# lmchion/PowerGridworld

Hardware: AMD Instinct MI355X
Metric: agent-env-steps/sec at batch 65536, 5-agent scenario, 1/2/4/8 MI355X (higher is better)
Workload: dtype f64; 1 GPU; C4: 5-agent coordinated buildings (building+PV+storage) + IEEE-13 power flow + voltage-violation reward; pf_convergence=opendss, batch_per_gpu=65536, global_batch=65536, episode_steps=286, parallelism=env-sharded x1 (no collective on the step path)

## Files before the change

include/pgw.h:

```cpp
#ifndef PGW_H_
#define PGW_H_

#include <stdint.h>

#ifdef __cplusplus
extern "C" {
#endif

#define PGW_ABI_VERSION 31

#define PGW_OK 0
#define PGW_ERR_ARG (-1)
#define PGW_ERR_HIP (-2)

int32_t pgw_abi_version(void);
const char* pgw_last_error(void);

#define PGW_N_STRUCT_SIZES 30
int32_t pgw_struct_sizes(int64_t* out, int32_t n);

typedef struct pgw_mat {
  double* ptr;
  int64_t s_env;
  int64_t s_dim;
} pgw_mat;

typedef struct pgw_matf {
  float* ptr;
  int64_t s_env;
  int64_t s_dim;
} pgw_matf;

#define PGW_OOB_EPS 1e-4

typedef struct pgw_battery_params {
  double soc_min, soc_max;
  double eta_c, eta_d;
  double max_power;
  double dt_h;
  int32_t rescale;
  int32_t sampled_init;
// ... 196 lines not shown
  const double* start;
  const double* resp;
  double resp_x0, resp_h;
  int32_t resp_nseg;
  int32_t resp_v_row;
  const double* resp_v;
  uint64_t resp_rows;
  const double* resp_q;
  uint64_t resp_q_rows;
  int32_t resp_q_stride, resp_q_k;
} pgw_pf_od;

int32_t pgw_pf_solve(const pgw_pf_params* p, const pgw_pf_tables* t, int64_t n,
                     const double* ctrl_p, const double* ctrl_q, double* v_out,
                     int32_t* iters, void* stream);
int32_t pgw_pf_solve_f32(const pgw_pf_params* p, const pgw_pf_tables* t, int64_t n,
                         const float* ctrl_p, const float* ctrl_q, float* v_out,
                         int32_t* iters, void* stream);

int64_t pgw_pf_od_probe_args_size(int32_t n_hours);
int32_t pgw_pf_od_probe(const pgw_pf_params* p_hours, int32_t n_hours, const pgw_pf_tables* t,
                        const double* start_h, int32_t lanes_per_hour, int64_t n, const double* P,
                        double* J_out, uint64_t* sig_out, int32_t* it_out, void* args_buf, void* stream);

int32_t pgw_pf_od_resp_fit(int32_t m, int64_t n_pieces, const double* J, const int32_t* idx3,
                           const double* meta, const int32_t* inext, const int32_t* rec, double* out,
                           void* stream);

int32_t pgw_pf_od_resp_check(int32_t m, int64_t n, const double* recs, const int32_t* rec, const double* P,
                             const double* J, const int32_t* iq, double* err, void* stream);

int32_t pgw_pf_pred_pack(const pgw_pf_params* p, int32_t n_tables, int32_t n_points,
                         const double* U_grid, double* rec, void* stream);
int32_t pgw_pf_pred_meta(const pgw_pf_params* p, int32_t n_tables, int32_t n_points,
                         const double* U_pred, const int32_t* sig, pgw_pred_meta* meta,
                         void* stream);

int32_t pgw_voltage_band_penalty(int64_t n, const double* v, double lo, double hi, double scale,
                                 double* out, void* stream);

int32_t pgw_pf_padded_m(int32_t m);
int64_t pgw_pf_pack_size(int32_t m);
int32_t pgw_pf_pack(const pgw_pf_params* p, const double* W, const double* U0, const double* G0,
                    const double* V0_0, double* out);

#define PGW_PFG_MAX_M 128
// ... 384 lines not shown
```

powergridworld_amd/_lib.py:

```python
import ctypes as C
import os

import torch

_HERE = os.path.dirname(os.path.abspath(__file__))
LIB_PATH = os.environ.get("PGW_LIB_PATH") or os.path.join(_HERE, "libpgw.so")
ABI_VERSION = 31

f64, i32, i64, u64, vp = C.c_double, C.c_int32, C.c_int64, C.c_uint64, C.c_void_p
P = C.POINTER

BLD_MAX_OBS = 24
EV_MAX_WORDS = 16
MAX_COMP = 8
PF_MAX_M = 16
PF_MAX_CTRL = 8
PFG_MAX_M = 128
PFG_MAX_CHK = 256
MAX_AGENTS = 8


class PgwError(RuntimeError):
    pass


class Mat(C.Structure):
    _fields_ = [("ptr", vp), ("s_env", i64), ("s_dim", i64)]


class Matf(C.Structure):
# ... 229 lines not shown
                ("soc_min", f64), ("soc_max", f64), ("eta_c", f64), ("eta_d", f64), ("max_power", f64),
                ("dt_h", f64), ("max_storage_cost", f64),
                ("ev_rate", f64), ("ev_hours_per_step", f64), ("ev_steps_per_hour", f64), ("ev_mult", f64),
                ("ev_unserved_penalty", f64), ("ev_obs_low", f64 * 7), ("ev_obs_high", f64 * 7),
                ("ev_end_park", f64 * HS_MAX_VEHICLES), ("ev_req0", f64 * HS_MAX_VEHICLES),
                ("dev_act_low", f64), ("dev_act_high", f64), ("dev_hours_per_step", f64),
                ("dev_obs_high", f64 * HS_MAX_DEV), ("max_grid_power", f64), ("oob", vp),
                ("pv_grid_aware", i32), ("pad_", i32)]


class HSStepInfo(C.Structure):
    _fields_ = [("pv_avail", f64), ("grid_cost", f64), ("dev_obs", f64 * HS_MAX_DEV),
                ("dev_power", f64 * HS_MAX_DEV), ("ev_time", f64), ("ev_next_time", f64),
                ("ev_window", C.c_uint64)]


class HSBuffers(C.Structure):
    _fields_ = [("action", Mat), ("obs", Mat), ("soc", vp), ("soc_cost", vp), ("ev_req", vp),
                ("ev_charging", vp), ("ev_cost", vp), ("dev_cost", vp), ("es_power_last", vp),
                ("reward", vp), ("real_power", vp), ("meta_out", vp), ("step_meta", vp),
                ("pv_power_last", vp), ("min_voltage", vp)]


PGW_ELEM_LINE, PGW_ELEM_XFMR, PGW_ELEM_VSOURCE, PGW_ELEM_SHUNT, PGW_ELEM_XFMR_N = 1, 2, 3, 4, 5

_SIGS = {
    "pgw_abi_version": (i32, []),
    "pgw_struct_sizes": (i32, [P(i64), i32]),
    "pgw_pf_od_probe_args_size": (i64, [i32]),
    "pgw_pf_od_probe": (i32, [P(PFParams), i32, P(PFTables), vp, i32, i64, vp, vp, vp, vp, vp, vp]),
    "pgw_pf_od_resp_fit": (i32, [i32, i64, vp, vp, vp, vp, vp, vp, vp]),
    "pgw_pf_od_resp_check": (i32, [i32, i64, vp, vp, vp, vp, vp, vp, vp]),
    "pgw_last_error": (C.c_char_p, []),
    "pgw_battery_reset": (i32, [P(BatteryParams), i64, vp, vp, Mat, vp]),
    "pgw_battery_step": (i32, [P(BatteryParams), i64, Mat, vp, Mat, vp, vp]),
    "pgw_battery_reset_f32": (i32, [P(BatteryParams), i64, vp, vp, Matf, vp]),
    "pgw_battery_step_f32": (i32, [P(BatteryParams), i64, Matf, vp, Matf, vp, vp]),
    "pgw_pv_obs": (i32, [P(PVParams), i64, f64, vp, Mat, vp]),
    "pgw_pv_step": (i32, [P(PVParams), i64, f64, Mat, vp, Mat, vp, vp]),
    "pgw_building_reset": (i32, [P(BuildingParams), P(BuildingExo), i64, vp, vp, vp, BuildingExt,
                                 Mat, vp]),
    "pgw_building_step": (i32, [P(BuildingParams), P(BuildingExo), P(BuildingExo), i64, Mat, vp, vp,
                                vp, vp, i32, BuildingExt, Mat, vp]),
    "pgw_ev_reset": (i32, [P(EVParams), i64, vp, vp, vp, vp]),
    "pgw_ev_reset_tables": (i32, [P(EVParams), i64, vp, vp, vp, vp]),
    "pgw_pv_obs_f32": (i32, [P(PVParams), i64, f64, vp, Matf, vp]),
    "pgw_pv_step_f32": (i32, [P(PVParams), i64, f64, Matf, vp, Matf, vp, vp]),
    "pgw_building_reset_f32": (i32, [P(BuildingParams), P(BuildingExo), i64, vp, vp, vp, BuildingExt, Matf, vp]),
    "pgw_building_step_f32": (i32, [P(BuildingParams), P(BuildingExo), P(BuildingExo), i64, Matf, vp, vp, vp, vp,
                                    i32, BuildingExt, Matf, vp]),
    "pgw_ev_reset_f32": (i32, [P(EVParams), i64, vp, vp, vp, vp]),
    "pgw_ev_reset_tables_f32": (i32, [P(EVParams), i64, vp, vp, vp, vp]),
    "pgw_ev_step_f32": (i32, [P(EVParams), P(EVStepInfo), i64, Matf, vp, vp, vp, Matf, vp, vp, vp]),
# ... 22 lines not shown
    "pgw_coord_step": (i32, [P(CoordParams), P(PFParams), P(PFTables), P(CoordStepInfo), i64,
                             CoordBuffers, vp]),
    "pgw_coord_step_f32": (i32, [P(CoordParams), P(PFParams), P(PFTables), P(CoordStepInfo), i64,
                                 CoordBuffersF32, vp]),
    "pgw_coord_step_general": (i32, [P(CoordParams), P(PFGParams), P(PFGTables), P(CoordStepInfo), i64,
                                     CoordBuffers, vp]),
    "pgw_hs_reset": (i32, [P(HSParams), P(HSStepInfo), i64, vp, HSBuffers, vp]),
    "pgw_mc_agent_step": (i32, [P(MCStepArgs), i64, vp]),
    "pgw_mc_agent_step_f32": (i32, [P(MCStepArgsF32), i64, vp]),
    "pgw_mc_ev_split_mode": (i32, [i32, P(i32)]),
    "pgw_graph_begin": (i32, [vp]),
    "pgw_graph_end": (i32, [vp, P(vp)]),
    "pgw_graph_launch": (i32, [vp, vp]),
    "pgw_graph_destroy": (i32, [vp]),
    "pgw_hs_step": (i32, [P(HSParams), P(HSStepInfo), i64, HSBuffers, vp]),
    "pgw_ma_step": (i32, [P(MAStepArgs), P(PFParams), P(PFTables), i64, vp, vp, vp]),
}

EXPORTED = sorted(_SIGS)

STRUCTS = [Mat, BatteryParams, PVParams, BuildingParams, BuildingExo, BuildingExt, EVParams,
           EVStepInfo, ReduceArgs, PFParams, PFTables, FeederElem, CoordParams, CoordBuffers,
           CoordStepInfo, PredMeta, HSParams, HSStepInfo, HSBuffers, MCStepArgs, Matf, CoordBuffersF32,
           MAStepArgs, PFGElem, PFGParams, PFGTables, RegParams, MCStepDyn, PFOD, MCStepArgsF32]

_lib = None


def lib():
    global _lib
    if _lib is not None:
        return _lib
    if not os.path.exists(LIB_PATH):
        raise PgwError("libpgw.so not found at %s -- build it with "
                       "`python -c 'import __graft_entry__ as g; g.build()'` or "
                       "`make -C powergridworld_amd/csrc`" % LIB_PATH)
    h = C.CDLL(LIB_PATH)
    for name, (res, args) in _SIGS.items():
        fn = getattr(h, name)
        fn.restype = res
        fn.argtypes = args
    if h.pgw_abi_version() != ABI_VERSION:
        raise PgwError("libpgw ABI %d != expected %d (rebuild)" % (h.pgw_abi_version(), ABI_VERSION))
    sizes = (i64 * len(STRUCTS))()
    h.pgw_struct_sizes(sizes, len(STRUCTS))
    for st, sz in zip(STRUCTS, sizes):
        if C.sizeof(st) != sz:
# ... 59 lines not shown
```

powergridworld_amd/csrc/pgw_feeder.cpp:

```cpp
#include <cmath>
#include <complex>
#include <cstdarg>
#include <cstdio>
#include <cstring>
#include <vector>

#include "pgw.h"

namespace pgw {
void set_error(const char* fmt, ...);
}

namespace {

using cplx = std::complex<double>;
using Mat = std::vector<cplx>;
using xcplx = std::complex<long double>;
using XMat = std::vector<xcplx>;

template <typename CT>
bool invert(std::vector<CT>& a, int n) {
  using R = typename CT::value_type;
  std::vector<CT> inv(static_cast<size_t>(n) * n, CT(0, 0));
  for (int i = 0; i < n; ++i) inv[i * n + i] = R(1);
// ... 208 lines not shown
  }
}

}

extern "C" {

int32_t pgw_struct_sizes(int64_t* out, int32_t n) {
  const int64_t sz[PGW_N_STRUCT_SIZES] = {
      (int64_t)sizeof(pgw_mat),           (int64_t)sizeof(pgw_battery_params),
      (int64_t)sizeof(pgw_pv_params),     (int64_t)sizeof(pgw_building_params),
      (int64_t)sizeof(pgw_building_exo),  (int64_t)sizeof(pgw_building_ext),
      (int64_t)sizeof(pgw_ev_params),     (int64_t)sizeof(pgw_ev_step_info),
      (int64_t)sizeof(pgw_reduce_args),   (int64_t)sizeof(pgw_pf_params),
      (int64_t)sizeof(pgw_pf_tables),     (int64_t)sizeof(pgw_feeder_elem),
      (int64_t)sizeof(pgw_coord_params),  (int64_t)sizeof(pgw_coord_buffers),
      (int64_t)sizeof(pgw_coord_step_info), (int64_t)sizeof(pgw_pred_meta),
      (int64_t)sizeof(pgw_hs_params),       (int64_t)sizeof(pgw_hs_step_info),
      (int64_t)sizeof(pgw_hs_buffers),      (int64_t)sizeof(pgw_mc_step_args),
      (int64_t)sizeof(pgw_matf),            (int64_t)sizeof(pgw_coord_buffers_f32),
      (int64_t)sizeof(pgw_ma_step_args),   (int64_t)sizeof(pgw_pfg_elem),
      (int64_t)sizeof(pgw_pfg_params),     (int64_t)sizeof(pgw_pfg_tables),
      (int64_t)sizeof(pgw_reg_params),    (int64_t)sizeof(pgw_mc_step_dyn),
      (int64_t)sizeof(pgw_pf_od),         (int64_t)sizeof(pgw_mc_step_args_f32)};
  for (int i = 0; i < n && i < PGW_N_STRUCT_SIZES; ++i) out[i] = sz[i];
  return PGW_N_STRUCT_SIZES;
}

int32_t pgw_feeder_build(const pgw_feeder_elem* elems, int32_t n_elems, int32_t n_nodes, double* Y,
                         double* Z, double* I_src, double* V0) {
  if (!elems || n_elems <= 0 || n_nodes <= 0) {
    pgw::set_error("pgw_feeder_build: empty feeder");
    return PGW_ERR_ARG;
  }
  try {
    Builder B(n_nodes);
    for (int i = 0; i < n_elems; ++i) {
      const pgw_feeder_elem& e = elems[i];
      if (e.nphases < 1 || e.nphases > 3) {
        pgw::set_error("pgw_feeder_build: element %d has %d phases", i, e.nphases);
        return PGW_ERR_ARG;
      }
      bool ok = false;
      switch (e.kind) {
        case PGW_ELEM_VSOURCE: ok = add_vsource(B, e); break;
        case PGW_ELEM_XFMR: ok = add_transformer(B, e); break;
        case PGW_ELEM_XFMR_N: ok = add_transformer_n(B, e); break;
// ... 99 lines not shown
```

powergridworld_amd/csrc/pgw_pf.hip:

```cpp
#include <algorithm>
#include <cstdlib>
#include <cmath>
#include <type_traits>
#include <atomic>
#include <vector>

#include "pgw_common.h"

static std::atomic<bool> g_pf_trace_on{false};

namespace pgw {

template <int B, int E, class F>
__device__ __forceinline__ void static_for(F&& f) {
  if constexpr (B < E) {
    f(std::integral_constant<int, B>{});
    static_for<B + 1, E>(f);
  }
}

template <int M> struct PFBlock {
  static constexpr int kTri = M * (M + 1) / 2;
  static constexpr int kU0re = 3 * kTri, kU0im = kU0re + M, kU0sum = kU0im + M;
  static constexpr int kLo2 = kU0sum + M, kMn2 = kLo2 + M, kMx2 = kMn2 + M;
  static constexpr int kG0re = kMx2 + M, kG0im = kG0re + M, kV0re = kG0im + M, kV0im = kV0re + 1;
  static constexpr int kSize = kV0im + 1;
  static constexpr int kPairs = (kSize + 15) / 16;
};
static int64_t pf_block_size(int m) { return 3LL * m * (m + 1) / 2 + 8LL * m + 2; }

// ... 2175 lines not shown
  __shared__ ODShared<M> sh;
  ODStage<M> stg;
  od_stage_load<M>(o, start, stg);
  PFSolver<M, true, false> S;
  S.load(a, t.block);
  double cp[PGW_PF_MAX_CTRL], cq[PGW_PF_MAX_CTRL];
#pragma unroll
  for (int c = 0; c < PGW_PF_MAX_CTRL; ++c) {
    cp[c] = (valid && c == 0) ? P[e] : 0.0;
    cq[c] = 0.0;
  }
  S.powers(a, cp, cq, 1.0);
  od_stage_store<M>(o, stg, sh);
  __syncthreads();
  uint64_t sig = kFnvBasis;
  const int it = od_solve<M, true>(S, o, stg, valid, sh, &sig);
  double ir[M], ii[M];
  od_load_J<M>(sh, it, ir, ii);
  if (!valid) return;
#pragma unroll
  for (int k = 0; k < M; ++k) J_out[e * M + k] = make_double2(ir[k], ii[k]);
  sig_out[e] = sig;
  it_out[e] = it;
}

__global__ void __launch_bounds__(kBlock) k_pf_od_resp_fit(int32_t m, int64_t np, const double2* __restrict__ J,
                                                           const int32_t* __restrict__ idx3,
                                                           const double* __restrict__ meta,
                                                           const int32_t* __restrict__ inext,
                                                           const int32_t* __restrict__ rec, double* __restrict__ out) {
  const int64_t i = (int64_t)blockIdx.x * kBlock + threadIdx.x;
  if (i >= np) return;
  double* o = out + (int64_t)rec[i] * PGW_OD_REC(m);
  for (int q = 0; q < 4; ++q) o[q] = meta[4 * i + q];
  const unsigned long long packed =
      (unsigned long long)(uint32_t)inext[2 * i] | ((unsigned long long)(uint32_t)inext[2 * i + 1] << 32);
  o[4] = __longlong_as_double((long long)packed);
  o[5] = 0.0;
  const double2* ja = J + (int64_t)idx3[3 * i] * m;
  const double2* jm = J + (int64_t)idx3[3 * i + 1] * m;
  const double2* jb = J + (int64_t)idx3[3 * i + 2] * m;
  double* c = o + PGW_OD_REC_HEAD;
  for (int k = 0; k < m; ++k) {
    const double2 a = ja[k], md = jm[k], b = jb[k];
    c[2 * k] = md.x;
    c[2 * k + 1] = md.y;
// ... 465 lines not shown
  PGW_REQUIRE(n_hours >= 1 && n >= 0 && lanes_per_hour > 0 && lanes_per_hour % kBlock == 0 &&
              n <= (int64_t)n_hours * lanes_per_hour,
              "pgw_pf_od_probe: n %lld lanes over %d hours of %d (a multiple of %d)", (long long)n, n_hours,
              lanes_per_hour, kBlock);
  std::vector<PFArgs> args(n_hours);
  for (int h = 0; h < n_hours; ++h) {
    const int32_t rc = check_od(p_hours[h], *t, "pgw_pf_od_probe");
    if (rc) return rc;
    PGW_REQUIRE(p_hours[h].m == p_hours[0].m && p_hours[h].n_ctrl == p_hours[0].n_ctrl &&
                p_hours[h].max_iter == p_hours[0].max_iter, "pgw_pf_od_probe: hours differ in shape");
    args[h] = make_pf_args(p_hours[h], *t);
  }
  if (n == 0) return PGW_OK;
  hipStream_t st = (hipStream_t)stream;
  PGW_REQUIRE(hipMemcpyAsync(args_buf, args.data(), sizeof(PFArgs) * n_hours, hipMemcpyHostToDevice, st) ==
                  hipSuccess && hipStreamSynchronize(st) == hipSuccess,
              "pgw_pf_od_probe: argument upload failed");
  hipLaunchKernelGGL(k_pf_od_probe<14>, dim3(grid_for(n)), dim3(kBlock), 0, st,
                     reinterpret_cast<const PFArgs*>(args_buf), make_od_args(*t->od, p_hours[0].max_iter), *t,
                     start_h, lanes_per_hour, n, P, reinterpret_cast<double2*>(J_out), sig_out, it_out);
  return check_launch("k_pf_od_probe");
}

int32_t pgw_pf_od_resp_fit(int32_t m, int64_t n_pieces, const double* J, const int32_t* idx3,
                           const double* meta, const int32_t* inext, const int32_t* rec, double* out,
                           void* stream) {
  PGW_REQUIRE(m >= 1 && m <= PGW_PF_MAX_M && n_pieces >= 0, "pgw_pf_od_resp_fit: bad m / n_pieces");
  if (n_pieces == 0) return PGW_OK;
  PGW_REQUIRE(J && idx3 && meta && inext && rec && out, "pgw_pf_od_resp_fit: null argument");
  hipLaunchKernelGGL(k_pf_od_resp_fit, dim3(grid_for(n_pieces)), dim3(kBlock), 0, (hipStream_t)stream, m,
                     n_pieces, reinterpret_cast<const double2*>(J), idx3, meta, inext, rec, out);
  return check_launch("k_pf_od_resp_fit");
}

int32_t pgw_pf_od_resp_check(int32_t m, int64_t n, const double* recs, const int32_t* rec, const double* P,
                             const double* J, const int32_t* iq, double* err, void* stream) {
  PGW_REQUIRE(m >= 1 && m <= PGW_PF_MAX_M && n >= 0, "pgw_pf_od_resp_check: bad m / n");
  if (n == 0) return PGW_OK;
  PGW_REQUIRE(recs && rec && P && J && iq && err, "pgw_pf_od_resp_check: null argument");
  hipLaunchKernelGGL(k_pf_od_resp_check, dim3(grid_for(n)), dim3(kBlock), 0, (hipStream_t)stream, m, n, recs,
                     rec, P, reinterpret_cast<const double2*>(J), iq, err);
  return check_launch("k_pf_od_resp_check");
}

int32_t pgw_pf_pred_meta(const pgw_pf_params* p, int32_t n_tables, int32_t n_points,
                         const double* U_pred, const int32_t* sig, pgw_pred_meta* meta,
// ... 137 lines not shown
```

powergridworld_amd/distribution_system/od_certify.py:

```python
import numpy as np
import torch

FNV_BASIS = np.uint64(0xcbf29ce484222325)
FNV_PRIME = np.uint64(0x100000001b3)


class SnapModel:

    def __init__(self, u1b, u1P, J0, jP, s0, fr, y0, u0, W, G, V0, lo2, mn2, mx2, tol, min_iter, max_iter):
        self.u1b, self.u1P, self.J0, self.jP = u1b, u1P, J0, jP
        self.s0, self.fr, self.y0, self.u0 = s0, fr, y0, u0
        self.W, self.G, self.V0 = W, G, V0
        self.Wa, self.Ga = W.abs(), G.abs()
        self.lo2, self.mn2, self.mx2 = float(lo2), float(mn2), float(mx2)
        self.tol, self.min_iter, self.max_iter = float(tol), int(min_iter), int(max_iter)

    @property
    def M(self):
        return self.u0.shape[0]

    @classmethod
    def from_solver(cls, s, rows, hours):
        M, dev = s.M, s.device
        st = s._od_start[torch.as_tensor(rows, device=dev)].to(torch.float64)
        c = torch.view_as_complex(st.reshape(len(rows), 6, M, 2).contiguous())
        p0, od = s.params, s._od_proto
        nph = np.array(p0.nph[:M])
        ctrl0 = np.array(p0.elem_ctrl[:M]) == 0
        s0 = []
        for h in hours:
            p = s._params_for_hour(h)
            s0.append((np.array(p.base_kw[:M]) * 1000.0) / nph - 1j * ((np.array(p.base_kvar[:M]) * 1000.0) / nph))
        T = lambda a: torch.as_tensor(np.ascontiguousarray(a), device=dev)
        return cls(u1b=c[:, 0], u1P=c[0, 1], J0=c[:, 3], jP=c[0, 4], s0=T(np.array(s0)),
                   fr=T(np.where(ctrl0, 1000.0 / nph, 0.0)),
                   y0=T(np.array(od.y0r[:M]) + 1j * np.array(od.y0i[:M])), u0=T(s._od_u0),
                   W=T(s._od_W2), G=T(s._od_Gall[:, :M]), V0=T(s._od_V0all),
                   lo2=p0.vlow[0] ** 2, mn2=p0.vmin[0] ** 2, mx2=p0.vmax[0] ** 2,
# ... 78 lines not shown
    rem = torch.where(gap > 0, e + ba * ba / (2.0 * torch.where(gap > 0, gap, torch.ones_like(gap))),
                      torch.full_like(aa, float("inf")))
    return aa, slope, rem


def _mul_cr(sa, sb, g0, g1, eg):
    a = sa * g0
    b = sa * g1 + sb * g0
    e = sb.abs() * g1.abs() + (sa.abs() + sb.abs()) * eg
    return a, b, e


def _mul_cc(x, y):
    xa, xb, xe = x
    ya, yb, ye = y
    a = xa * ya
    b = xa * yb + xb * ya
    e = xb.abs() * yb.abs() + (xa.abs() + xb.abs()) * ye + (ya.abs() + yb.abs()) * xe + xe * ye
    return a, b, e


def certify(model, h, lo, hi, delta_band=1e-12, delta_stop=1e-12):
    dev = model.u0.device
    h = torch.as_tensor(h, device=dev)
    lo = torch.as_tensor(lo, dtype=torch.float64, device=dev)
    hi = torch.as_tensor(hi, dtype=torch.float64, device=dev)
    K, M = lo.shape[0], model.M
    c, r = (0.5 * (lo + hi))[:, None], (0.5 * (hi - lo))[:, None]
    zero_e = torch.zeros((K, M), dtype=torch.float64, device=dev)
    u = (model.u1b[h] + c * model.u1P, r * model.u1P, zero_e)
    Jp = (model.J0[h] + c * model.jP, r * model.jP, zero_e)
    Vp = _lin(Jp, model.G, model.Ga, model.V0)
    s_a = model.s0[h] + (c * model.fr).to(torch.complex128)
    s_b = (r * model.fr).to(torch.complex128)
    ok = torch.ones(K, dtype=torch.bool, device=dev)
    done = torch.zeros(K, dtype=torch.bool, device=dev)
    conv = torch.zeros_like(done)
    its = torch.ones(K, dtype=torch.int64, device=dev)
    shifts = 2 * torch.arange(M, device=dev)
    thr = (model.lo2, model.mn2, model.mx2)
    bands = []
    for it in range(2, model.max_iter + 1):
        m0, m1, em, mlo, mhi = _mag2(u)
        b = torch.zeros((K, M), dtype=torch.int64, device=dev)
        for T in thr:
            above, below = mlo > T + delta_band, mhi < T - delta_band
            ok &= done | (above | below).all(1)
            b += above.long()
        bands.append(torch.where(done, -1, (b << shifts).sum(1)))
        inband = b == 2
        safe = torch.where(inband, m0, torch.ones_like(m0))
        g0 = torch.where(inband, 1.0 / safe,
                         torch.where(b == 1, 1.0 / model.mn2, torch.where(b == 3, 1.0 / model.mx2, 1.0)))
        g1 = torch.where(inband, -m1 / (safe * safe), torch.zeros_like(m1))
        mlo_s = torch.where(inband, mlo, torch.ones_like(mlo))
        eg = torch.where(inband, em / (safe * safe) + (m1.abs() + em) ** 2 / (safe * safe * mlo_s),
                         torch.zeros_like(em))
        ok &= done | torch.isfinite(eg).all(1)
        ya, yb, ye = _mul_cr(s_a, s_b, g0, g1, eg)
        J = _mul_cc((ya - model.y0, yb, ye), u)
        V = _lin(J, model.G, model.Ga, model.V0)
        un = _lin(J, model.W, model.Wa, model.u0)
        n0, n1, nr = _mag(V)
        p0, p1, pr = _mag(Vp)
        d0, d1, dr = n0 - p0, n1 - p1, nr + pr
        dlo, dhi = d0 - d1.abs() - dr, d0 + d1.abs() + dr
        amax = torch.maximum(dlo.abs(), dhi.abs())
        amin = torch.where((dlo <= 0) & (dhi >= 0), torch.zeros_like(dlo), torch.minimum(dlo.abs(), dhi.abs()))
        if it >= model.min_iter:
            yes = (amax <= model.tol - delta_stop).all(1)
            no = (amin > model.tol + delta_stop).any(1)
        else:
            yes = torch.zeros_like(done)
            no = torch.ones_like(done)
        ok &= done | yes | no
        its = torch.where(done, its, torch.full_like(its, it))
        conv |= ~done & yes
        done = done | yes | (it >= model.max_iter) | ~ok
        u = tuple(torch.where(done[:, None], x_o, x_n) for x_o, x_n in zip(u, un))
        Vp = V
        if bool(done.all()):
            break
    ret = torch.where(conv, its, -its)
    return ok.cpu().numpy(), ret.cpu().numpy(), signature(torch.stack(bands, 1), ret)


def certify_pieces(model, h, a, b, it, sig, min_width=1e-9, max_depth=12, max_live=64, split=16):
    h, a, b = np.asarray(h), np.asarray(a, float), np.asarray(b, float)
    it, sig = np.asarray(it, np.int64), np.asarray(sig, np.uint64)
    n = len(a)
    out_lo, out_hi, kw = np.full(n, np.inf), np.full(n, -np.inf), np.zeros(n)
    if n == 0:
        return out_lo, out_hi, kw
    owner, lo, hi = np.arange(n), a.copy(), b.copy()
    good = {}
    for level in range(max_depth):
        if not len(owner):
            break
        ok, ret, sg = certify(model, h[owner], lo, hi)
        ok &= (ret == it[owner]) & (sg == sig[owner])
        if level == 0:
            out_lo[ok], out_hi[ok], kw[ok] = a[ok], b[ok], b[ok] - a[ok]
        else:
            for q in np.nonzero(ok)[0]:
                good.setdefault(owner[q], []).append((lo[q], hi[q]))
        bad = np.nonzero(~ok & (hi - lo > split * min_width))[0]
        if max_live:
# ... 26 lines not shown
```

powergridworld_amd/distribution_system/opendss.py:

```python
import os
from datetime import datetime
from typing import List, Union

import numpy as np
import pandas as pd
import torch

from powergridworld_amd import _lib
from powergridworld_amd.base import as_env_tensor
from powergridworld_amd.distribution_system.feeder import DATA_DIR, Feeder, load_feeder_spec
from powergridworld_amd.distribution_system.powerflow import PowerFlowSolver

PHASE_MAP = {'a': '.1', 'b': '.2', 'c': '.3'}


def bus_name_to_nodes(bus_name: str) -> List[str]:
    if bus_name[-1] in PHASE_MAP.keys():
        return [bus_name.replace(bus_name[-1], PHASE_MAP[bus_name[-1]])]
    return [bus_name + p for p in PHASE_MAP.values()]


def load_loadshape(loadshape_file):
    base = os.path.basename(str(loadshape_file)).lower()
    if base == "annual_hourly_load_profile.csv" and not os.path.exists(str(loadshape_file)):
# ... 221 lines not shown
        od.gamma = max([float(np.abs(Gs[j] - Gs[r]).max()) for j, r in members], default=0.0)
        od.eps = max([float(abs(V0s[j] - V0s[r])) for j, r in members], default=0.0)
        od.gmax = float(rowmax[elem_nodes + reps].max())
        od.gsrc = float(rowmax[src].max()) if src else 0.0
        dev = self.device
        cdev = lambda a: torch.tensor(np.ascontiguousarray(a).view(np.float64).ravel(), dtype=torch.float64,
                                      device=dev)
        self._od_Gall, self._od_V0all = Gs, V0s
        self._od_rows_V0 = cdev(V0s[rows] if rows else np.zeros(1, complex))
        self._od_rows_G = cdev(Gs[rows] if rows else np.zeros((1, M), complex))
        od.rows_V0, od.rows_G = self._od_rows_V0.data_ptr(), self._od_rows_G.data_ptr()
        self._od_proto = od
        self._od_rows = [f.node_names[i] for i in rows]
        self._od_W2 = W / (vb_elem[:, None] * vb_elem[None, :])
        self._od_u0 = U0 / vb_elem
        self._od_start = torch.zeros((self.OD_MAX_TABLES, 12 * M), dtype=torch.float64, device=dev)
        self._od_resp = None
        self._od_vresp = None
        self._od_rowmask = {}
        self.od_node_records = True
        self.od_row_masks = True
        self.od_record_rows = True
        self.od_certify = True
        self.od_row_records = True
        self._od_qrec = None
        self._od_qinfo = {}
        self._od_qflags = {}
        self.od_resp_stats, self.od_resp_brackets = {}, {}
        self._od_index = {}
        self._od_keep = {}

    def _od_starts(self, hour):
        hours, keys = [], []
        for h in range(hour, min(hour + self.PREDICTOR_LOOKAHEAD, len(self.annual_hourly_load_profile))):
            k = self._hour_key(h)
            if k not in self._od_index and k not in keys:
                hours.append(h)
                keys.append(k)
        if len(self._od_index) + len(keys) > self.OD_MAX_TABLES:
            self._od_index, self._tables_cache, self._od_keep = {}, {}, {}
            self.tables_version += 1
        idx0 = len(self._od_index)
        M, od = self.M, self._od_proto
        W2, u0 = self._od_W2, self._od_u0
        p0 = self.params
        nph = np.array(p0.nph[:M])
# ... 310 lines not shown
        err = torch.empty(2 * len(pa), dtype=torch.float64, device=dev)
        dr, dp, dq_ = T(np.repeat(prec, 2), np.int32), T(chk.ravel(), np.float64), T(c_l.ravel(), np.int32)
        _lib.check(lib.pgw_pf_od_resp_check(M, 2 * len(pa), self._od_resp.data_ptr(), dr.data_ptr(), dp.data_ptr(),
                                            Jc.data_ptr(), dq_.data_ptr(), err.data_ptr(), st))
        e_ = err.cpu().numpy().reshape(-1, 2).max(1)
        del dr, dp, dq_
        vnode = self._od_vnode()
        if vnode is not None and len(pa):
            rr = self._od_resp.view(-1, R)[torch.from_numpy(prec).to(dev)]
            vc = self._od_vcoef(rr)
            tt = (torch.from_numpy(chk).to(dev) - rr[:, 2:3]) * rr[:, 3:4]
            vfit = vc[:, :1] + tt * (vc[:, 1:2] + tt * vc[:, 2:3])
            Jl = torch.view_as_complex(Jc.reshape(-1, M, 2)[torch.from_numpy(c_l.ravel()).to(dev)].contiguous())
            G = torch.from_numpy(np.ascontiguousarray(self._od_Gall[vnode, :M])).to(dev)
            vtrue = ((Jl * G).sum(-1) + complex(self._od_V0all[vnode])).reshape(-1, 2)
            ev = ((vfit - vtrue).abs() / vtrue.abs()).max(1).values.cpu().numpy()
            e_ = np.maximum(e_, np.where(np.isfinite(ev), ev, np.inf))
        bad = (pit != 0) & ((e_ > self.OD_RESP_TOL) | (sc[c_l] != psig[:, None]).any(1) | ~np.isfinite(e_))
        cand = np.nonzero((pit != 0) & ~bad)[0]
        n_cut, kw_cut, t_cert = 0, 0.0, _time.perf_counter()
        if self.od_certify and len(cand):
            from powergridworld_amd.distribution_system.od_certify import SnapModel, certify_pieces
            model = SnapModel.from_solver(self, list(range(idx0, idx0 + H)), hours)
            c_lo, c_hi, c_kw = certify_pieces(model, pq_[cand], pa[cand], pb[cand], pit[cand], psig[cand],
                                              min_width=self.OD_RESP_MIN_WIDTH)
            none = c_lo > c_hi
            bad[cand[none]] = True
            cut = ~none & ((c_lo > pa[cand]) | (c_hi < pb[cand]))
            n_cut = int(cut.sum())
            kw_cut = float(((pb - pa)[cand] - np.where(none, 0.0, c_hi - c_lo)).sum())
            if n_cut:
                hdr = torch.from_numpy(np.stack([c_lo[cut], c_hi[cut]], 1)).to(dev)
                self._od_resp.view(-1, R)[torch.from_numpy(prec[cand[cut]]).to(dev), 0:2] = hdr
        t_cert = _time.perf_counter() - t_cert
        if bad.any():
            words = np.array([self._od_meta_word(0, int(nx)) for nx in pnext[bad]], np.int64)
            self._od_resp.view(-1, R).view(torch.int64)[torch.from_numpy(prec[bad]).to(dev), 4] = \
                torch.from_numpy(words).to(dev)
        ok = (pit != 0) & ~bad
        if vnode is not None:
            if self._od_vresp is None:
                self._od_vresp = torch.zeros((self.OD_MAX_TABLES, rec_n, _lib.OD_VREC), dtype=torch.float64,
                                             device=dev)
            vb = self._od_vresp[idx0:idx0 + H]
            vb.view(torch.int64)[:, :, :6] = blk.view(torch.int64)[:, :, :6]
            vb[:, :, 6:12] = torch.view_as_real(self._od_vcoef(blk)).reshape(H, rec_n, 6)
# ... 639 lines not shown
```

Before: 15.65 billion agent-env-steps/s.

## Port interval power-flow certification to a fused native HIP kernel

Adds a HIP kernel that runs the per-interval affine-arithmetic fixed-point certification entirely per lane, with per-node previous magnitudes kept in LDS. It replaces the iterative PyTorch implementation, which launched many small tensor ops per iteration, whenever the model lives on a GPU. The certification runs during OpenDSS response-table construction, not inside the per-step environment kernel. So any gain shows up only through table-building overhead that is amortized over steps. It adds an ABI bump and a hardcoded m=14, and results could differ slightly from the torch path.

```diff
diff --git a/include/pgw.h b/include/pgw.h
--- a/include/pgw.h
+++ b/include/pgw.h
@@ -7,7 +7,7 @@
 extern "C" {
 #endif
 
-#define PGW_ABI_VERSION 31
+#define PGW_ABI_VERSION 32
 
 #define PGW_OK 0
 #define PGW_ERR_ARG (-1)
@@ -16,7 +16,7 @@
 int32_t pgw_abi_version(void);
 const char* pgw_last_error(void);
 
-#define PGW_N_STRUCT_SIZES 30
+#define PGW_N_STRUCT_SIZES 31
 int32_t pgw_struct_sizes(int64_t* out, int32_t n);
 
 typedef struct pgw_mat {
@@ -259,6 +259,16 @@
 int32_t pgw_pf_od_probe(const pgw_pf_params* p_hours, int32_t n_hours, const pgw_pf_tables* t,
                         const double* start_h, int32_t lanes_per_hour, int64_t n, const double* P,
                         double* J_out, uint64_t* sig_out, int32_t* it_out, void* args_buf, void* stream);
+
+typedef struct pgw_od_certify_model {
+  const double *u1b, *u1P, *J0, *jP, *s0, *fr, *y0, *u0, *W, *Wa, *G, *Ga, *V0;
+  double lo2, mn2, mx2, tol, delta_band, delta_stop;
+  int32_t m, n_nodes, n_hours, min_iter, max_iter, pad_;
+} pgw_od_certify_model;
+#define PGW_OD_CERTIFY_MAX_NODES 42
+
+int32_t pgw_pf_od_certify(const pgw_od_certify_model* model, int64_t k, const int32_t* h, const double* lo,
+                          const double* hi, int32_t* ok, int32_t* ret, uint64_t* sig, void* stream);
 
 int32_t pgw_pf_od_resp_fit(int32_t m, int64_t n_pieces, const double* J, const int32_t* idx3,
                            const double* meta, const int32_t* inext, const int32_t* rec, double* out,
diff --git a/powergridworld_amd/_lib.py b/powergridworld_amd/_lib.py
--- a/powergridworld_amd/_lib.py
+++ b/powergridworld_amd/_lib.py
@@ -5,7 +5,7 @@
 
 _HERE = os.path.dirname(os.path.abspath(__file__))
 LIB_PATH = os.environ.get("PGW_LIB_PATH") or os.path.join(_HERE, "libpgw.so")
-ABI_VERSION = 31
+ABI_VERSION = 32
 
 f64, i32, i64, u64, vp = C.c_double, C.c_int32, C.c_int64, C.c_uint64, C.c_void_p
 P = C.POINTER
@@ -281,6 +281,14 @@
                 ("pv_power_last", vp), ("min_voltage", vp)]
 
 
+class ODCertifyModel(C.Structure):
+    _fields_ = [(k, vp) for k in ("u1b", "u1P", "J0", "jP", "s0", "fr", "y0", "u0", "W", "Wa", "G", "Ga", "V0")] + \
+               [(k, f64) for k in ("lo2", "mn2", "mx2", "tol", "delta_band", "delta_stop")] + \
+               [(k, i32) for k in ("m", "n_nodes", "n_hours", "min_iter", "max_iter", "pad_")]
+
+
+OD_CERTIFY_MAX_NODES = 42
+
 PGW_ELEM_LINE, PGW_ELEM_XFMR, PGW_ELEM_VSOURCE, PGW_ELEM_SHUNT, PGW_ELEM_XFMR_N = 1, 2, 3, 4, 5
 
 _SIGS = {
@@ -288,6 +296,7 @@
     "pgw_struct_sizes": (i32, [P(i64), i32]),
     "pgw_pf_od_probe_args_size": (i64, [i32]),
     "pgw_pf_od_probe": (i32, [P(PFParams), i32, P(PFTables), vp, i32, i64, vp, vp, vp, vp, vp, vp]),
+    "pgw_pf_od_certify": (i32, [P(ODCertifyModel), i64, vp, vp, vp, vp, vp, vp, vp]),
     "pgw_pf_od_resp_fit": (i32, [i32, i64, vp, vp, vp, vp, vp, vp, vp]),
     "pgw_pf_od_resp_check": (i32, [i32, i64, vp, vp, vp, vp, vp, vp, vp]),
     "pgw_last_error": (C.c_char_p, []),
@@ -356,7 +365,8 @@
 STRUCTS = [Mat, BatteryParams, PVParams, BuildingParams, BuildingExo, BuildingExt, EVParams,
            EVStepInfo, ReduceArgs, PFParams, PFTables, FeederElem, CoordParams, CoordBuffers,
            CoordStepInfo, PredMeta, HSParams, HSStepInfo, HSBuffers, MCStepArgs, Matf, CoordBuffersF32,
-           MAStepArgs, PFGElem, PFGParams, PFGTables, RegParams, MCStepDyn, PFOD, MCStepArgsF32]
+           MAStepArgs, PFGElem, PFGParams, PFGTables, RegParams, MCStepDyn, PFOD, MCStepArgsF32,
+           ODCertifyModel]
 
 _lib = None
 
diff --git a/powergridworld_amd/csrc/pgw_feeder.cpp b/powergridworld_amd/csrc/pgw_feeder.cpp
--- a/powergridworld_amd/csrc/pgw_feeder.cpp
+++ b/powergridworld_amd/csrc/pgw_feeder.cpp
@@ -254,7 +254,8 @@
       (int64_t)sizeof(pgw_ma_step_args),   (int64_t)sizeof(pgw_pfg_elem),
       (int64_t)sizeof(pgw_pfg_params),     (int64_t)sizeof(pgw_pfg_tables),
       (int64_t)sizeof(pgw_reg_params),    (int64_t)sizeof(pgw_mc_step_dyn),
-      (int64_t)sizeof(pgw_pf_od),         (int64_t)sizeof(pgw_mc_step_args_f32)};
+      (int64_t)sizeof(pgw_pf_od),         (int64_t)sizeof(pgw_mc_step_args_f32),
+      (int64_t)sizeof(pgw_od_certify_model)};
   for (int i = 0; i < n && i < PGW_N_STRUCT_SIZES; ++i) out[i] = sz[i];
   return PGW_N_STRUCT_SIZES;
 }
diff --git a/powergridworld_amd/csrc/pgw_od_certify.h b/powergridworld_amd/csrc/pgw_od_certify.h
--- /dev/null
+++ b/powergridworld_amd/csrc/pgw_od_certify.h
@@ -0,0 +1,176 @@
+#pragma once
+#include <math.h>
+#include <stdint.h>
+
+#include "pgw.h"
+
+#ifdef __HIPCC__
+#define PGW_CERT_HD __host__ __device__ __forceinline__
+#else
+#define PGW_CERT_HD inline
+#endif
+
+PGW_CERT_HD double cert_max(double x, double y) { return (x != x || y != y) ? NAN : (x > y ? x : y); }
+PGW_CERT_HD double cert_min(double x, double y) { return (x != x || y != y) ? NAN : (x < y ? x : y); }
+
+PGW_CERT_HD void cert_mag(double ar, double ai, double br, double bi, double e, double& m0, double& m1,
+                          double& rem) {
+#pragma clang fp contract(off)
+  const double aa = hypot(ar, ai), ba = hypot(br, bi);
+  m1 = (ar * br + ai * bi) / (aa > 0.0 ? aa : 1.0);
+  const double gap = aa - ba;
+  rem = gap > 0.0 ? e + ba * ba / (2.0 * gap) : (double)INFINITY;
+  m0 = aa;
+}
+
+template <int M>
+PGW_CERT_HD void cert_row(const double* __restrict__ mat, const double* __restrict__ mabs,
+                          const double* __restrict__ cst, int n, const double* xar, const double* xai,
+                          const double* xbr, const double* xbi, const double* xe, double& ar, double& ai,
+                          double& br, double& bi, double& e) {
+#pragma clang fp contract(off)
+  const double* g = mat + 2 * (int64_t)n * M;
+  const double* ga = mabs + (int64_t)n * M;
+  double sar = 0.0, sai = 0.0, sbr = 0.0, sbi = 0.0, se = 0.0;
+#pragma unroll
+  for (int j = 0; j < M; ++j) {
+    const double gr = g[2 * j], gi = g[2 * j + 1];
+    sar += xar[j] * gr - xai[j] * gi;
+    sai += xar[j] * gi + xai[j] * gr;
+    sbr += xbr[j] * gr - xbi[j] * gi;
+    sbi += xbr[j] * gi + xbi[j] * gr;
+    se += xe[j] * ga[j];
+  }
+  ar = cst[2 * n] + sar;
+  ai = cst[2 * n + 1] + sai;
+  br = sbr;
+  bi = sbi;
+  e = se;
+}
+
+template <int M>
+PGW_CERT_HD void od_certify_lane(const pgw_od_certify_model& a, int h, double lo, double hi,
+                                 double* __restrict__ prev, int stride, int32_t* ok_out, int32_t* ret_out,
+                                 uint64_t* sig_out) {
+#pragma clang fp contract(off)
+  const int N = a.n_nodes;
+  const double c = 0.5 * (lo + hi), r = 0.5 * (hi - lo);
+  const double thr[3] = {a.lo2, a.mn2, a.mx2};
+  const double tol_yes = a.tol - a.delta_stop, tol_no = a.tol + a.delta_stop;
+  const double* u1b = a.u1b + 2 * (int64_t)h * M;
+  const double* J0 = a.J0 + 2 * (int64_t)h * M;
+  const double* s0 = a.s0 + 2 * (int64_t)h * M;
+  double uar[M], uai[M], ubr[M], ubi[M], ue[M];
+  double jar[M], jai[M], jbr[M], jbi[M], je[M];
+#pragma unroll
+  for (int k = 0; k < M; ++k) {
+    uar[k] = u1b[2 * k] + c * a.u1P[2 * k];
+    uai[k] = u1b[2 * k + 1] + c * a.u1P[2 * k + 1];
+    ubr[k] = r * a.u1P[2 * k];
+    ubi[k] = r * a.u1P[2 * k + 1];
+    ue[k] = 0.0;
+    jar[k] = J0[2 * k] + c * a.jP[2 * k];
+    jai[k] = J0[2 * k + 1] + c * a.jP[2 * k + 1];
+    jbr[k] = r * a.jP[2 * k];
+    jbi[k] = r * a.jP[2 * k + 1];
+    je[k] = 0.0;
+  }
+#pragma unroll 1
+  for (int n = 0; n < N; ++n) {
+    double var, vai, vbr, vbi, ve, p0, p1, pr;
+    cert_row<M>(a.G, a.Ga, a.V0, n, jar, jai, jbr, jbi, je, var, vai, vbr, vbi, ve);
+    cert_mag(var, vai, vbr, vbi, ve, p0, p1, pr);
+    prev[(3 * n + 0) * (int64_t)stride] = p0;
+    prev[(3 * n + 1) * (int64_t)stride] = p1;
+    prev[(3 * n + 2) * (int64_t)stride] = pr;
+  }
+  bool ok = true, conv = false;
+  int its = 1;
+  uint64_t sig = 0xcbf29ce484222325ull;
+  const uint64_t prime = 0x100000001b3ull;
+  for (int it = 2; it <= a.max_iter; ++it) {
+    uint64_t bands = 0;
+    bool certain = true;
+#pragma unroll
+    for (int k = 0; k < M; ++k) {
+      const double ar = uar[k], ai = uai[k], br = ubr[k], bi = ubi[k], e = ue[k];
+      const double m0 = ar * ar + ai * ai;
+      const double m1 = 2.0 * (ar * br + ai * bi);
+      const double q2 = br * br + bi * bi;
+      const double qmax = m0 + fabs(m1) + q2;
+      const double q2s = q2 > 0.0 ? q2 : 1.0;
+      const double tv = q2 > 0.0 ? -m1 / (2.0 * q2s) : 0.0;
+      const bool inside = q2 > 0.0 && fabs(tv) <= 1.0;
+      double qmin = inside ? m0 - m1 * m1 / (4.0 * q2s) : m0 - fabs(m1) + q2;
+      qmin = qmin < 0.0 ? 0.0 : qmin;
+      double rlo = sqrt(qmin) - e;
+      rlo = rlo < 0.0 ? 0.0 : rlo;
+      const double mlo = rlo * rlo;
+      const double rhi = sqrt(qmax) + e;
+      const double mhi = rhi * rhi;
+      const double aa = hypot(ar, ai), ba = hypot(br, bi);
+      const double em = q2 + 2.0 * (aa + ba) * e + e * e;
+      int b = 0;
+#pragma unroll
+      for (int q = 0; q < 3; ++q) {
+        const bool above = mlo > thr[q] + a.delta_band, below = mhi < thr[q] - a.delta_band;
+        certain &= above | below;
+        b += above ? 1 : 0;
+      }
+      bands |= (uint64_t)b << (2 * k);
+      const bool inband = b == 2;
+      const double safe = inband ? m0 : 1.0;
+      const double g0 = inband ? 1.0 / safe : (b == 1 ? 1.0 / a.mn2 : (b == 3 ? 1.0 / a.mx2 : 1.0));
+      const double g1 = inband ? -m1 / (safe * safe) : 0.0;
+      const double mlo_s = inband ? mlo : 1.0;
+      const double w = fabs(m1) + em;
+      const double eg = inband ? em / (safe * safe) + w * w / (safe * safe * mlo_s) : 0.0;
+      certain &= (bool)isfinite(eg);
+      const double sar = s0[2 * k] + c * a.fr[k], sai = s0[2 * k + 1] + 0.0, sbr = r * a.fr[k];
+      const double sa_abs = hypot(sar, sai), sb_abs = fabs(sbr);
+      const double yar = sar * g0 - a.y0[2 * k], yai = sai * g0 - a.y0[2 * k + 1];
+      const double ybr = sar * g1 + sbr * g0, ybi = sai * g1 + 0.0;
+      const double ye = sb_abs * fabs(g1) + (sa_abs + sb_abs) * eg;
+      jar[k] = yar * ar - yai * ai;
+      jai[k] = yar * ai + yai * ar;
+      jbr[k] = (yar * br - yai * bi) + (ybr * ar - ybi * ai);
+      jbi[k] = (yar * bi + yai * br) + (ybr * ai + ybi * ar);
+      const double ya_abs = hypot(yar, yai), yb_abs = hypot(ybr, ybi);
+      je[k] = yb_abs * ba + (ya_abs + yb_abs) * e + (aa + ba) * ye + ye * e;
+    }
+    ok &= certain;
+    sig = (sig ^ bands) * prime;
+    bool yes = true, no = false;
+#pragma unroll 1
+    for (int n = 0; n < N; ++n) {
+      double var, vai, vbr, vbi, ve, n0, n1, nr;
+      cert_row<M>(a.G, a.Ga, a.V0, n, jar, jai, jbr, jbi, je, var, vai, vbr, vbi, ve);
+      cert_mag(var, vai, vbr, vbi, ve, n0, n1, nr);
+      double* p = prev + 3 * n * (int64_t)stride;
+      const double d0 = n0 - p[0], d1 = n1 - p[stride], dr = nr + p[2 * (int64_t)stride];
+      const double dlo = d0 - fabs(d1) - dr, dhi = d0 + fabs(d1) + dr;
+      const double amax = cert_max(fabs(dlo), fabs(dhi));
+      const double amin = (dlo <= 0.0 && dhi >= 0.0) ? 0.0 : cert_min(fabs(dlo), fabs(dhi));
+      yes &= amax <= tol_yes;
+      no |= amin > tol_no;
+      p[0] = n0;
+      p[stride] = n1;
+      p[2 * (int64_t)stride] = nr;
+    }
+    if (it < a.min_iter) {
+      yes = false;
+      no = true;
+    }
+    ok &= yes | no;
+    its = it;
+    conv |= yes;
+    if (yes || it >= a.max_iter || !ok) break;
+#pragma unroll
+    for (int k = 0; k < M; ++k)
+      cert_row<M>(a.W, a.Wa, a.u0, k, jar, jai, jbr, jbi, je, uar[k], uai[k], ubr[k], ubi[k], ue[k]);
+  }
+  const int32_t ret = conv ? its : -its;
+  *ok_out = ok ? 1 : 0;
+  *ret_out = ret;
+  *sig_out = (sig ^ (uint64_t)(uint32_t)ret) * prime;
+}
diff --git a/powergridworld_amd/csrc/pgw_pf.hip b/powergridworld_amd/csrc/pgw_pf.hip
--- a/powergridworld_amd/csrc/pgw_pf.hip
+++ b/powergridworld_amd/csrc/pgw_pf.hip
@@ -6,6 +6,7 @@
 #include <vector>
 
 #include "pgw_common.h"
+#include "pgw_od_certify.h"
 
 static std::atomic<bool> g_pf_trace_on{false};
 
@@ -2227,6 +2228,27 @@
   for (int k = 0; k < M; ++k) J_out[e * M + k] = make_double2(ir[k], ii[k]);
   sig_out[e] = sig;
   it_out[e] = it;
+}
+
+constexpr int kCertBlock = 64;
+template <int M>
+__global__ void __launch_bounds__(kCertBlock) k_pf_od_certify(pgw_od_certify_model a, int64_t K,
+                                                              const int32_t* __restrict__ h,
+                                                              const double* __restrict__ lo,
+                                                              const double* __restrict__ hi,
+                                                              int32_t* __restrict__ ok, int32_t* __restrict__ ret,
+                                                              uint64_t* __restrict__ sig) {
+  extern __shared__ double cert_prev[];
+  const int64_t e = (int64_t)blockIdx.x * kCertBlock + threadIdx.x;
+  if (e >= K) return;
+  const int row = h[e];
+  if (row < 0 || row >= a.n_hours) {
+    ok[e] = 0;
+    ret[e] = 0;
+    sig[e] = 0;
+    return;
+  }
+  od_certify_lane<M>(a, row, lo[e], hi[e], cert_prev + threadIdx.x, kCertBlock, ok + e, ret + e, sig + e);
 }
 
 __global__ void __launch_bounds__(kBlock) k_pf_od_resp_fit(int32_t m, int64_t np, const double2* __restrict__ J,
@@ -2738,6 +2760,26 @@
   return check_launch("k_pf_od_probe");
 }
 
+int32_t pgw_pf_od_certify(const pgw_od_certify_model* model, int64_t k, const int32_t* h, const double* lo,
+                          const double* hi, int32_t* ok, int32_t* ret, uint64_t* sig, void* stream) {
+  PGW_REQUIRE(model && k >= 0, "pgw_pf_od_certify: null model / negative k");
+  const pgw_od_certify_model& a = *model;
+  PGW_REQUIRE(a.m == 14 && a.n_nodes >= 1 && a.n_nodes <= PGW_OD_CERTIFY_MAX_NODES && a.n_hours >= 1 &&
+              a.max_iter >= 2,
+              "pgw_pf_od_certify: m %d (14), n_nodes %d (1..%d), n_hours %d, max_iter %d (>= 2)", a.m, a.n_nodes,
+              PGW_OD_CERTIFY_MAX_NODES, a.n_hours, a.max_iter);
+  PGW_REQUIRE(a.u1b && a.u1P && a.J0 && a.jP && a.s0 && a.fr && a.y0 && a.u0 && a.W && a.Wa && a.G && a.Ga && a.V0,
+              "pgw_pf_od_certify: null model array");
+  if (k == 0) return PGW_OK;
+  PGW_REQUIRE(h && lo && hi && ok && ret && sig, "pgw_pf_od_certify: null argument");
+  const int64_t blocks = (k + kCertBlock - 1) / kCertBlock;
+  PGW_REQUIRE(blocks <= 0x7fffffffll, "pgw_pf_od_certify: %lld intervals", (long long)k);
+  const size_t lds = sizeof(double) * 3 * (size_t)a.n_nodes * kCertBlock;
+  hipLaunchKernelGGL(k_pf_od_certify<14>, dim3((unsigned)blocks), dim3(kCertBlock), lds, (hipStream_t)stream, a, k,
+                     h, lo, hi, ok, ret, sig);
+  return check_launch("k_pf_od_certify");
+}
+
 int32_t pgw_pf_od_resp_fit(int32_t m, int64_t n_pieces, const double* J, const int32_t* idx3,
                            const double* meta, const int32_t* inext, const int32_t* rec, double* out,
                            void* stream) {
diff --git a/powergridworld_amd/distribution_system/od_certify.py b/powergridworld_amd/distribution_system/od_certify.py
--- a/powergridworld_amd/distribution_system/od_certify.py
+++ b/powergridworld_amd/distribution_system/od_certify.py
@@ -14,6 +14,25 @@
         self.Wa, self.Ga = W.abs(), G.abs()
         self.lo2, self.mn2, self.mx2 = float(lo2), float(mn2), float(mx2)
         self.tol, self.min_iter, self.max_iter = float(tol), int(min_iter), int(max_iter)
+        self.native = True
+        self._native = None
+
+    def native_model(self, delta_band, delta_stop):
+        from powergridworld_amd import _lib
+        if self._native is None:
+            ri = lambda z: torch.view_as_real(z.to(torch.complex128).contiguous()).contiguous()
+            re = lambda x: x.to(torch.float64).contiguous()
+            arrays = dict(u1b=ri(self.u1b), u1P=ri(self.u1P), J0=ri(self.J0), jP=ri(self.jP), s0=ri(self.s0),
+                          fr=re(self.fr), y0=ri(self.y0), u0=ri(self.u0), W=ri(self.W), Wa=re(self.Wa),
+                          G=ri(self.G), Ga=re(self.Ga), V0=ri(self.V0))
+            m = _lib.ODCertifyModel(m=self.M, n_nodes=self.G.shape[0], n_hours=self.u1b.shape[0],
+                                    **{k: v.data_ptr() for k, v in arrays.items()})
+            self._native = (m, arrays)
+        m = self._native[0]
+        m.lo2, m.mn2, m.mx2, m.tol = self.lo2, self.mn2, self.mx2, self.tol
+        m.min_iter, m.max_iter = self.min_iter, self.max_iter
+        m.delta_band, m.delta_stop = float(delta_band), float(delta_stop)
+        return m
 
     @property
     def M(self):
@@ -138,6 +157,8 @@
 
 def certify(model, h, lo, hi, delta_band=1e-12, delta_stop=1e-12):
     dev = model.u0.device
+    if model.native and dev.type == "cuda":
+        return _certify_native(model, h, lo, hi, delta_band, delta_stop)
     h = torch.as_tensor(h, device=dev)
     lo = torch.as_tensor(lo, dtype=torch.float64, device=dev)
     hi = torch.as_tensor(hi, dtype=torch.float64, device=dev)
@@ -166,8 +187,9 @@
         bands.append(torch.where(done, -1, (b << shifts).sum(1)))
         inband = b == 2
         safe = torch.where(inband, m0, torch.ones_like(m0))
+        one = torch.ones_like(m0)
         g0 = torch.where(inband, 1.0 / safe,
-                         torch.where(b == 1, 1.0 / model.mn2, torch.where(b == 3, 1.0 / model.mx2, 1.0)))
+                         torch.where(b == 1, one * (1.0 / model.mn2), torch.where(b == 3, one * (1.0 / model.mx2), one)))
         g1 = torch.where(inband, -m1 / (safe * safe), torch.zeros_like(m1))
         mlo_s = torch.where(inband, mlo, torch.ones_like(mlo))
         eg = torch.where(inband, em / (safe * safe) + (m1.abs() + em) ** 2 / (safe * safe * mlo_s),
@@ -199,6 +221,27 @@
             break
     ret = torch.where(conv, its, -its)
     return ok.cpu().numpy(), ret.cpu().numpy(), signature(torch.stack(bands, 1), ret)
+
+
+def _certify_native(model, h, lo, hi, delta_band, delta_stop):
+    from powergridworld_amd import _lib
+    host = lambda x, dt: (x.detach().cpu().numpy() if torch.is_tensor(x) else np.asarray(x)).astype(dt)
+    h, lo, hi = host(h, np.int32), host(lo, np.float64), host(hi, np.float64)
+    K, dev = lo.shape[0], model.u0.device
+    if K == 0:
+        return np.zeros(0, bool), np.zeros(0, np.int64), np.zeros(0, np.uint64)
+    inp = np.empty((3, K), np.float64)
+    inp[0], inp[1] = lo, hi
+    inp[2].view(np.int32)[:K] = h
+    d_in = torch.from_numpy(inp).to(dev)
+    d_out = torch.empty((2, K), dtype=torch.int64, device=dev)
+    i32 = d_out[1].view(torch.int32)
+    _lib.check(_lib.lib().pgw_pf_od_certify(model.native_model(delta_band, delta_stop), K, d_in[2].data_ptr(),
+                                            d_in[0].data_ptr(), d_in[1].data_ptr(), i32[:K].data_ptr(),
+                                            i32[K:].data_ptr(), d_out[0].data_ptr(), _lib.stream_ptr(dev)))
+    out = d_out.cpu().numpy()
+    okret = out[1].view(np.int32)
+    return okret[:K] != 0, okret[K:].astype(np.int64), out[0].view(np.uint64).copy()
 
 
 def certify_pieces(model, h, a, b, it, sig, min_width=1e-9, max_depth=12, max_live=64, split=16):
diff --git a/powergridworld_amd/distribution_system/opendss.py b/powergridworld_amd/distribution_system/opendss.py
--- a/powergridworld_amd/distribution_system/opendss.py
+++ b/powergridworld_amd/distribution_system/opendss.py
@@ -267,6 +267,7 @@
         self.od_row_masks = True
         self.od_record_rows = True
         self.od_certify = True
+        self.od_certify_native = True
         self.od_row_records = True
         self._od_qrec = None
         self._od_qinfo = {}
@@ -623,6 +624,7 @@
         if self.od_certify and len(cand):
             from powergridworld_amd.distribution_system.od_certify import SnapModel, certify_pieces
             model = SnapModel.from_solver(self, list(range(idx0, idx0 + H)), hours)
+            model.native = bool(self.od_certify_native)
             c_lo, c_hi, c_kw = certify_pieces(model, pq_[cand], pa[cand], pb[cand], pit[cand], psig[cand],
                                               min_width=self.OD_RESP_MIN_WIDTH)
             none = c_lo > c_hi
```

Measured after the change: 16.17 billion agent-env-steps/s, median of 6. +3.3%, better.
